# clayjohn/godot-volumetric-cloud-demo-v2

Measured on AMD Instinct MI355X. Metric: Mrays/s + hemisphere fps, 2048x1024 @ 128x6 steps, 1/2/4/8 MI355X, higher is better.
Workload: dtype f32

## Files before the change

godot-volumetric-cloud-demo-v2_amd/csrc/api.cpp:

```cpp
#include <cstdarg>
#include <cstdio>
#include <cstdlib>
#include <cstring>
#include <new>
#include <algorithm>
#include <vector>
#include "context.h"
#include "bake_core.h"
#include "mip_args.h"
#include "cloud_core.h"
#include "order_core.h"
#include "primitives_core.h"

using namespace csky;

__attribute__((constructor)) static void csky_runtime_defaults() {
    const char* no = getenv("CSKY_NO_ENV");
    if (no && no[0] && no[0] != '0') return;
    if (!getenv("GPU_MAX_HW_QUEUES")) setenv("GPU_MAX_HW_QUEUES", "16", 0);
}

static_assert(sizeof(csky_cloud_params) == sizeof(CloudParams), "ABI struct mismatch");

namespace {
// ... 33 lines not shown
    hs.d.reset(); hs.h.reset();
    if ((rc = hs.d.alloc(c, px))) return rc;
    return hs.h.alloc(c, px * 8);
}

}

extern "C" {

int csky_abi_version(void) { return CSKY_ABI_VERSION; }

int csky_device_count(void) {
    int n = 0;
    if (hipGetDeviceCount(&n) != hipSuccess) return 0;
    return n;
}

const char* csky_last_error(const csky_ctx* ctx) { return ctx ? ctx->err : g_err; }
const char* csky_last_warning(const csky_ctx* ctx) { return ctx ? ctx->warn : ""; }

int csky_create(csky_ctx** out, int device_id) {
    if (!out) return fail(nullptr, CSKY_ERR_INVALID, "csky_create: out is NULL");
    *out = nullptr;
    int n = 0;
    hipError_t e = hipGetDeviceCount(&n);
    if (e != hipSuccess || n <= 0)
        return fail(nullptr, CSKY_ERR_NO_DEVICE, "csky_create: no HIP device available (%s); libcloudsky has no CPU fallback",
                    e == hipSuccess ? "device count is 0" : hipGetErrorString(e));
    if (device_id < 0 || device_id >= n) return fail(nullptr, CSKY_ERR_INVALID, "csky_create: device_id %d out of range [0,%d)", device_id, n);
    csky_ctx* c = new (std::nothrow) csky_ctx();
    if (!c) return fail(nullptr, CSKY_ERR_INVALID, "csky_create: out of host memory");
    c->device = device_id;
    if (const int rc = create_resources(c)) { fail(nullptr, rc, "csky_create: %s", c->err); csky_destroy(c); return rc; }
    { int cus = 0; (void)hipDeviceGetAttribute(&cus, hipDeviceAttributeMultiprocessorCount, device_id); c->resident_wgs = (cus > 0 ? cus : 256) * cloud_resident_workgroups_per_cu(); }
    if (const char* pe = getenv("CSKY_PERSISTENT")) c->persistent = atoi(pe);
    if (const char* pe = getenv("CSKY_PERSISTENT_WGS")) { const int n = atoi(pe); if (n > 0) c->resident_wgs = n; }
    *out = c;
    return CSKY_OK;
}

void csky_destroy(csky_ctx* c) {
    if (!c) return;
    (void)hipSetDevice(c->device);
    (void)hipDeviceSynchronize();
    delete c;
}

#ifdef CSKY_BRICK_BOUND
static int upload_brick_bounds(csky_ctx* c, const uint8_t* large_rgba8) {
    std::vector<float> tab(16 * 16 * 16);
    for (int bz = 0; bz < 16; bz++) for (int by = 0; by < 16; by++) for (int bx = 0; bx < 16; bx++) {
        int rm = 0, fm = 1 << 30;
        for (int z = bz * 8; z <= bz * 8 + 8; z++) for (int y = by * 8; y <= by * 8 + 8; y++) for (int x = bx * 8; x <= bx * 8 + 8; x++) {
            const uint8_t* tx = large_rgba8 + ((((size_t)(z & 127) * 128 + (y & 127)) * 128 + (x & 127)) * 4);
            rm = std::max(rm, (int)tx[0]); fm = std::min(fm, 5 * tx[1] + 2 * tx[2] + tx[3]);
        }
        const float r = rm * (1.0f / 255.0f), f = fm * (1.0f / (8.0f * 255.0f));
        tab[((size_t)bz * 16 + by) * 16 + bx] = (r + (1.0f - f)) / (2.0f - f) * 1.000004f;
    }
    if (const int rc = c->noise.d_brick.grow(c, tab.size())) return rc;
    HIPCHK(c, hipMemcpy(c->noise.d_brick, tab.data(), tab.size() * sizeof(float), hipMemcpyHostToDevice));
    return CSKY_OK;
}
#endif

static int set_noise(csky_ctx* c, const uint8_t* large_rgba8, const uint8_t* small_rgb8, const uint8_t* weather_rgb8, bool chains_given) {
    if (!c) return fail(nullptr, CSKY_ERR_INVALID, "csky_set_noise: ctx is NULL");
    if (!large_rgba8 || !small_rgb8 || !weather_rgb8) return fail(c, CSKY_ERR_INVALID, "csky_set_noise: NULL texture pointer");
    int rc; if ((rc = bind(c))) return rc;
// ... 445 lines not shown
```

godot-volumetric-cloud-demo-v2_amd/csrc/cloud_kernels.hip:

```cpp
#include <hip/hip_runtime.h>
#include "kernels.h"
#include "cloud_core.h"
#include "order_core.h"
#include <type_traits>
#pragma clang fp contract(off)

namespace csky {

constexpr int QCAP = 96;
constexpr int QSTEPS = 48;
constexpr int Q_FLOATS = 5 * QCAP + 7 * QCAP + 3 * QSTEPS;

__device__ __forceinline__ void wave_lds_fence() {
    __builtin_amdgcn_fence(__ATOMIC_RELEASE, "wavefront");
    __builtin_amdgcn_wave_barrier();
    __builtin_amdgcn_fence(__ATOMIC_ACQUIRE, "wavefront");
}

__device__ __forceinline__ float ray_phase(const FrameConsts& fc, const Ray& ray) {
    float phase = 0.0f;
    if (ray.above) {
        const float ct = fc.ldir[0] * ray.dx + fc.ldir[1] * ray.dy + fc.ldir[2] * ray.dz;
        phase = fmaxf(fmaxf(henyey_greenstein(ct, 0.6f), henyey_greenstein(ct, fc.hg_g2)), henyey_greenstein(ct, -0.2f));
    }
// ... 71 lines not shown
        }
        if (count <= QCAP - 64 && cs < QSTEPS && i + 1 < step_end) continue;
        if (count == 0) continue;
        wave_lds_fence();
        light_march_batch(T, fc, ls, count, lane, [&](int k, float& x, float& y, float& z) { x = ev_px[k]; y = ev_py[k]; z = ev_pz[k]; }, ev_lt, QCAP);
        wave_lds_fence();
        for (int s = 0; s < cs; s++) {
            const unsigned lo = st_lo[s], hi = st_hi[s];
            const bool mine = lane < 32 ? ((lo >> lane) & 1u) : ((hi >> (lane - 32)) & 1u);
            if (mine) {
                const int slot = (int)st_base[s] + (int)__builtin_amdgcn_mbcnt_hi(hi, __builtin_amdgcn_mbcnt_lo(lo, 0u));
                float cd = 0.0f;
                for (int j = 0; j < nl; j++) cd += ev_lt[j * QCAP + slot];
                const float et = ev_t[slot], ehf = ev_hf[slot];
                const float dt = fast_exp(nd * et * ray.ss);
                shade_sample(fc, phase, et, ehf, dt, cd, Tr, alpha, Lr, Lg, Lb);
                o.incloud++;
            }
        }
        wave_lds_fence();
        count = 0; cs = 0;
        if (fc.early_eps > 0.0f) {
            if (Tr < fc.early_eps) live = false;
            if (!__any(live)) break;
        }
    }
    o.r = Lr; o.g = Lg; o.b = Lb; o.a = sat(alpha); o.t = Tr;
    return o;
}

constexpr int CQ_CAP = 128;
constexpr int CQ_STEPS = 66;
constexpr int CQ_FLOATS = 5 * CQ_CAP + CQ_CAP / 4 + 3 * CQ_STEPS + 2 + 128 + 320;

#ifndef CSKY_EAGER_LIGHT
#define CSKY_EAGER_LIGHT 1
#endif
#if CSKY_EAGER_LIGHT
#define CSKY_LIGHT_SAMPLE(CT) sample_density_eager<true, false, CT>
#else
#define CSKY_LIGHT_SAMPLE(CT) sample_density<CT>
#endif
#ifndef CSKY_EAGER_PRIMARY
#define CSKY_EAGER_PRIMARY 0
#endif
#if CSKY_EAGER_PRIMARY == 1
#define CSKY_PRIMARY_SAMPLE(CT) sample_density_eager<false, false, CT>
#elif CSKY_EAGER_PRIMARY == 2
#define CSKY_PRIMARY_SAMPLE(CT) sample_density_eager<true, false, CT>
#else
#define CSKY_PRIMARY_SAMPLE(CT) sample_density<CT>
#endif
#ifndef CSKY_LIGHT_STRAIGHT
#define CSKY_LIGHT_STRAIGHT 1
#endif
#if CSKY_EAGER_LIGHT
template <int CT, int J, class TS>
__device__ __forceinline__ void light_samples_from(const TS& T, const FrameConsts& fc, const int ls, float& lx, float& ly, float& lz, float& cd) {
    if constexpr (J < 6) {
        if (J >= ls) return;
        advance(lx, ly, lz, fc.linc[J][0], fc.linc[J][1], fc.linc[J][2]);
        const float lhf = height_fraction(length3_shell(lx, ly, lz));
        cd += sample_density_eager<true, (J > 2), CT>(T, fc, lx, ly, lz, lhf, fc.wpos_x, fc.wpos_y, J > 2 ? J - 2 : 0, J);
        light_samples_from<CT, J + 1>(T, fc, ls, lx, ly, lz, cd);
    }
}
// ... 14 lines not shown
        for (int j = 0; j < JS; j++) {
            if (j >= ls) break;
            advance(lx, ly, lz, fc.linc[j][0], fc.linc[j][1], fc.linc[j][2]);
            const float lhf = height_fraction(length3_shell(lx, ly, lz));
            cd += CSKY_LIGHT_SAMPLE(CT)(T, fc, lx, ly, lz, lhf, fc.wpos_x, fc.wpos_y, j > 2 ? j - 2 : 0, j);
        }
    }
#if CSKY_EAGER_LIGHT
    if constexpr (STRAIGHT) {
        light_samples_from<CT, 0>(T, fc, ls, lx, ly, lz, cd);
    } else if constexpr (TS::small_detail) {
#pragma unroll 1
        for (int j = JS; j < 6; j++) {
            if (j >= ls) break;
            advance(lx, ly, lz, fc.linc[j][0], fc.linc[j][1], fc.linc[j][2]);
            const float lhf = height_fraction(length3_shell(lx, ly, lz));
            cd += sample_density_eager<true, true, CT>(T, fc, lx, ly, lz, lhf, fc.wpos_x, fc.wpos_y, j - 2, j);
        }
    }
#endif
    {
        lx = ex; ly = ey; lz = ez;
        advance(lx, ly, lz, fc.ldist[0], fc.ldist[1], fc.ldist[2]);
        const float lhf = height_fraction(length3_shell(lx, ly, lz));
        const float ld = CSKY_LIGHT_SAMPLE(CT)(T, fc, lx, ly, lz, lhf, 0.0f, 0.0f, 3, 5);
        cd += fast_pow(ld, (1.0f - lhf) * 0.8f + 0.5f);
    }
    float et, ehf, ess, eph;
    late(et, ehf, ess, eph);
    dt = fast_exp(nd * et * ess);
    shade_terms(fc, eph, et, ehf, dt, cd, Dr, Dg, Db, rq);
}

template <bool WHOLE, bool TALLY, int CT = 0, class TS, bool RISING = true>
__device__ __forceinline__ MarchOut march_compact(const TS& T, const FrameConsts& fc, Ray ray, float* __restrict__ q, int step_begin, int step_end) {
    constexpr bool SAT = WHOLE && !TS::cell32;
    constexpr bool DEAD = SAT && !TALLY;
    float* __restrict__ ev_px = q;
    float* __restrict__ ev_py = q + CQ_CAP;
    float* __restrict__ ev_pz = q + 2 * CQ_CAP;
    float* __restrict__ ev_t = q + 3 * CQ_CAP;
    float* __restrict__ ev_hf = q + 4 * CQ_CAP;
    unsigned char* __restrict__ ev_owner = reinterpret_cast<unsigned char*>(q + 5 * CQ_CAP);
    unsigned* __restrict__ st_lo = reinterpret_cast<unsigned*>(q + 5 * CQ_CAP + CQ_CAP / 4);
    unsigned* __restrict__ st_hi = st_lo + CQ_STEPS;
    unsigned* __restrict__ st_base = st_hi + CQ_STEPS;

    MarchOut o; o.r = o.g = o.b = o.a = 0.0f; o.t = 1.0f; o.incloud = 0;
    const int lane = threadIdx.x & 63;
    const int ls = fc.light_steps;
    const float phase = ray_phase(fc, ray);
    float px = ray.px, py = ray.py, pz = ray.pz;
    const float nd = -fc.density;
    bool live = ray.above;
    int count = 0, cs = 0;
    bool latched = false;
    unsigned skipped = 0u;
    unsigned* __restrict__ tally = st_base + CQ_STEPS;
    if constexpr (TALLY) { if (lane == 0) tally[0] = 0u; }
    float* __restrict__ ray_ss = reinterpret_cast<float*>(tally + 2);
    float* __restrict__ ray_ph = ray_ss + 64;
    ray_ss[lane] = ray.ss; ray_ph[lane] = phase;
    float* __restrict__ acc = ray_ph + 64;
    acc[lane] = 1.0f; acc[64 + lane] = 0.0f; acc[128 + lane] = 0.0f; acc[192 + lane] = 0.0f; acc[256 + lane] = 0.0f;
    if (__builtin_amdgcn_ballot_w64(live) == 0ull) return o;
    for (int i = 0; i < step_begin; i++) advance(px, py, pz, ray.sx, ray.sy, ray.sz);
    int end = step_end;
    for (int i = step_begin;;) {
        if (i < end) {
            float t, hf;
            bool have = false, below_top = false;
            if (live) {
                advance(px, py, pz, ray.sx, ray.sy, ray.sz);
                hf = height_fraction(length3_shell(px, py, pz));
                t = CSKY_PRIMARY_SAMPLE(CT)(T, fc, px, py, pz, hf, fc.wpos_x, fc.wpos_y, 0, 0);
                have = t > 0.0f;
                below_top = !(hf >= fc.hf_hi);
            }
            if constexpr (SAT && TALLY) {
                skipped += (unsigned)__popcll(__builtin_amdgcn_ballot_w64(have && latched));
                have = have && !latched;
            }
            if constexpr (RISING) {
                if ((i & 3) == 3 && __builtin_amdgcn_ballot_w64(below_top) == 0ull) end = i + 1;
            } else {
                if ((i & 3) == 3 && __builtin_amdgcn_ballot_w64(live) == 0ull) end = i + 1;
            }
            const unsigned long long m = __builtin_amdgcn_ballot_w64(have);
            if (m != 0ull) {
                const int slot = count + (int)__builtin_amdgcn_mbcnt_hi((unsigned)(m >> 32), __builtin_amdgcn_mbcnt_lo((unsigned)m, 0u));
                if (have) { ev_px[slot] = px; ev_py[slot] = py; ev_pz[slot] = pz; ev_t[slot] = t; ev_hf[slot] = hf; ev_owner[slot] = (unsigned char)lane; }
                if (lane == 0) { st_lo[cs] = (unsigned)m; st_hi[cs] = (unsigned)(m >> 32); st_base[cs] = (unsigned)count; }
                count += __popcll(m);
                cs++;
            }
            i++;
        }
        const bool last = i >= end;
        if (count == 0) { if (last) break; continue; }
        if (count < 64 && !last) continue;
        wave_lds_fence();
        const int n = count < 64 ? count : 64;
        unsigned long long carry = 0ull;
        if constexpr (TALLY) { if (lane == 0) tally[0] += (unsigned)n; }
        if (lane < n) {
            float Dr, Dg, Db, rq, dt;
            light_march_terms<CT>(T, fc, ls, nd, ev_px[lane], ev_py[lane], ev_pz[lane],
                              [&](float& et, float& ehf, float& ess, float& eph) { et = ev_t[lane]; ehf = ev_hf[lane]; const int ow = ev_owner[lane]; ess = ray_ss[ow]; eph = ray_ph[ow]; }, Dr, Dg, Db, rq, dt);
            ev_px[lane] = Dr; ev_py[lane] = Dg; ev_pz[lane] = Db; ev_t[lane] = rq; ev_hf[lane] = dt;
        }
        wave_lds_fence();
        float Tr = acc[lane], alpha = acc[64 + lane], Lr = acc[128 + lane], Lg = acc[192 + lane], Lb = acc[256 + lane];
        for (int s = 0; s < cs; s++) {
            const unsigned lo = (unsigned)__builtin_amdgcn_readfirstlane((int)st_lo[s]), hi = (unsigned)__builtin_amdgcn_readfirstlane((int)st_hi[s]);
            const bool mine = __builtin_amdgcn_inverse_ballot_w64(((unsigned long long)hi << 32) | lo);
            const int slot = (int)st_base[s] + (int)__builtin_amdgcn_mbcnt_hi(hi, __builtin_amdgcn_mbcnt_lo(lo, 0u));
            if (mine && slot < n) {
                composite_sample(ev_hf[slot], ev_t[slot], ev_px[slot], ev_py[slot], ev_pz[slot], Tr, alpha, Lr, Lg, Lb);
            }
            if (s == cs - 1) carry = __builtin_amdgcn_ballot_w64(mine && slot >= n);
        }
        if constexpr (DEAD) {
            const bool cand = live && alpha >= SAT_ALPHA_MIN;
            if (fc.sat_skip != 0 && __builtin_amdgcn_ballot_w64(cand) != 0ull) {
                float B[3];
                ray_saturation_bound(fc, ray_ph[lane], B);
                const float L[3] = {Lr, Lg, Lb};
                if (cand && ray_saturated(fc, Tr, alpha, L, B)) live = false;
            }
        } else if constexpr (SAT) {
            const bool cand = !latched && alpha >= SAT_ALPHA_MIN;
            if (fc.sat_skip != 0 && __builtin_amdgcn_ballot_w64(cand) != 0ull) {
                float B[3];
                ray_saturation_bound(fc, ray_ph[lane], B);
                const float L[3] = {Lr, Lg, Lb};
                latched = latched || (cand && ray_saturated(fc, Tr, alpha, L, B));
            }
        }
        acc[lane] = Tr; acc[64 + lane] = alpha; acc[128 + lane] = Lr; acc[192 + lane] = Lg; acc[256 + lane] = Lb;
        wave_lds_fence();
        const int rem = count - n;
        if (rem > 0) {
            float a0 = 0.0f, a1 = 0.0f, a2 = 0.0f, a3 = 0.0f, a4 = 0.0f; unsigned char a5 = 0;
            if (lane < rem) { a0 = ev_px[n + lane]; a1 = ev_py[n + lane]; a2 = ev_pz[n + lane]; a3 = ev_t[n + lane]; a4 = ev_hf[n + lane]; a5 = ev_owner[n + lane]; }
            wave_lds_fence();
            if (lane < rem) { ev_px[lane] = a0; ev_py[lane] = a1; ev_pz[lane] = a2; ev_t[lane] = a3; ev_hf[lane] = a4; ev_owner[lane] = a5; }
            if (lane == 0) { st_lo[0] = (unsigned)carry; st_hi[0] = (unsigned)(carry >> 32); st_base[0] = 0u; }
            wave_lds_fence();
            count = rem; cs = 1;
        } else {
            count = 0; cs = 0;
        }
        if (fc.early_eps > 0.0f) {
            if (Tr < fc.early_eps) live = false;
            if (__builtin_amdgcn_ballot_w64(live) == 0ull) break;
        }
        if (last && count == 0) break;
    }
    wave_lds_fence();
    o.r = acc[128 + lane]; o.g = acc[192 + lane]; o.b = acc[256 + lane]; o.a = sat(acc[64 + lane]); o.t = acc[lane];
    if constexpr (TALLY) o.incloud = lane == 0 ? tally[0] + skipped : 0u;
    return o;
}


struct Pixel { int gx, gy, lr; bool valid; };
__device__ __forceinline__ Pixel footprint_pixel(const RenderGeom& G, const uint32_t logical, const int tiles_x, const int bw, const int tile, const int lane) {
    const int local_rows = G.n_bands * G.band_rows;
    const int slab = (int)logical / tiles_x, bx = (int)logical - slab * tiles_x;
    Pixel p;
    p.gx = bx * bw + tile * 8 + (lane & 7);
    p.lr = slab * 8 + (lane >> 3);
    p.valid = p.gx < G.tile_w && p.lr < local_rows;
    const int band = p.lr / G.band_rows, rib = p.lr - band * G.band_rows;
    p.gy = (G.first_band + band * G.band_stride) * G.band_rows + rib;
    return p;
}
__device__ __forceinline__ void store_pixel(uint2* __restrict__ out, const RenderGeom& G, int gx, int gy, int lr, float r, float g, float b, float a) {
    out[(size_t)(G.out_full ? gy : lr) * G.pitch_px + gx] = pack_half4(f2h(r), f2h(g), f2h(b), f2h(a));
}
// ... 122 lines not shown
    {
        const uint4* __restrict__ src = reinterpret_cast<const uint4*>(T.detail_h);
        uint4* dst = reinterpret_cast<uint4*>(lds_all);
        for (int i = threadIdx.x; i < DETAIL_FLOATS / 4; i += 1024) dst[i] = src[i];
    }
    __syncthreads();
    const uint32_t logical = order[blockIdx.x];
    if (logical == 0xffffffffu) return;
    const int wave = threadIdx.x >> 6, lane = threadIdx.x & 63;
    const Pixel pix = footprint_pixel(G, logical, (G.tile_w + 127) >> 7, 128, wave, lane);
    const bool valid = pix.valid;
    const FrameConsts& fc = *fcp;
    Ray ray = ray_setup(fc, valid ? pix.gx : 0, valid ? pix.gy : 0);
    if (!valid) ray.above = false;
    TexSet Tl = T;
    Tl.detail_lds = detail_s;
    const MarchOut o = march_queue(Tl, fc, ray, queues + wave * Q_FLOATS, 0, fc.primary_steps);
    if (valid) {
        store_pixel(out, G, pix.gx, pix.gy, pix.lr, o.r, o.g, o.b, o.a);
    }
    if (stats || wg_cost) {
        unsigned ic = o.incloud, ab = ray.above ? 1u : 0u;
        for (int off = 32; off > 0; off >>= 1) { ic += __shfl_down(ic, off); ab += __shfl_down(ab, off); }
        if (lane == 0) {
            if (stats) { atomicAdd(&stats[0], (unsigned long long)ic); atomicAdd(&stats[1], (unsigned long long)ab); }
            if (wg_cost) atomicAdd(&wg_cost[logical], ic + 16u * ab);
        }
    }
}

#ifndef CSKY_COMPACT_WAVES
#define CSKY_COMPACT_WAVES 7
#endif
template <int VARIANT, int SEG, class TS = TexSet, bool TALLY = true, int CT = 0>
__device__ __forceinline__ void render_block(TS T, const FrameConsts* __restrict__ fcp, const RenderGeom& G, const uint32_t logical, const uint32_t rec,
                                             uint2* __restrict__ out, unsigned long long* __restrict__ stats, uint32_t* __restrict__ wg_cost, const int tile_of_wave = -1) {
    constexpr int BW = 32 / SEG;
    const int tiles_x = (G.tile_w + BW - 1) / BW;
    const int local_rows = G.n_bands * G.band_rows;
    const int slab = (int)logical / tiles_x, bx = (int)logical - slab * tiles_x;
    const int wave = threadIdx.x >> 6, lane = threadIdx.x & 63;
    const int tile = tile_of_wave >= 0 ? tile_of_wave : wave / SEG, seg = tile_of_wave >= 0 ? 0 : wave - tile * SEG;
    const int gx = bx * BW + tile * 8 + (lane & 7);
    const int lr = slab * 8 + (lane >> 3);
    const bool valid = gx < G.tile_w && lr < local_rows;
    const int band = lr / G.band_rows, rib = lr - band * G.band_rows;
    const int gy = (G.first_band + band * G.band_stride) * G.band_rows + rib;

    const FrameConsts& fc = *fcp;
    T.detail_lds = nullptr;
    Ray ray = ray_setup(fc, valid ? gx : 0, valid ? gy : 0);
    if (!valid) ray.above = false;
    MarchOut o;
    if constexpr (VARIANT == 0) {
        static_assert(SEG == 1, "the lock-step reference variant marches whole rays");
        o = march(T, fc, ray);
    } else {
        __shared__ float lds[4][VARIANT == 3 ? CQ_FLOATS : Q_FLOATS];
        const int s0 = (fc.primary_steps * seg) / SEG, s1 = (fc.primary_steps * (seg + 1)) / SEG;
        if constexpr (VARIANT == 3) o = march_compact<SEG == 1, TALLY, CT>(T, fc, ray, &lds[wave][0], s0, s1);
        else o = march_queue(T, fc, ray, &lds[wave][0], s0, s1);
        if constexpr (SEG > 1) {
            __shared__ float comb[4][5][64];
            comb[wave][0][lane] = o.r; comb[wave][1][lane] = o.g; comb[wave][2][lane] = o.b; comb[wave][3][lane] = o.t; comb[wave][4][lane] = o.a;
            __syncthreads();
            if (seg == 0) {
                float Tr = o.t, na = 1.0f - o.a;
#pragma unroll
                for (int s = 1; s < SEG; s++) {
                    const int w = tile * SEG + s;
                    o.r += Tr * comb[w][0][lane]; o.g += Tr * comb[w][1][lane]; o.b += Tr * comb[w][2][lane];
                    Tr *= comb[w][3][lane]; na *= 1.0f - comb[w][4][lane];
                }
                o.a = sat(1.0f - na); o.t = Tr;
            }
        }
    }
    if (valid && seg == 0) {
        store_pixel(out, G, gx, gy, lr, o.r, o.g, o.b, o.a);
    }
    if constexpr (TALLY) {
    if (stats || wg_cost) {
        unsigned ic = o.incloud, ab = (ray.above && seg == 0) ? 1u : 0u;
        for (int off = 32; off > 0; off >>= 1) { ic += __shfl_down(ic, off); ab += __shfl_down(ab, off); }
        if (lane == 0) {
            if (stats) { atomicAdd(&stats[0], (unsigned long long)ic); atomicAdd(&stats[1], (unsigned long long)ab); }
            if (wg_cost) atomicAdd(&wg_cost[logical], ic + 16u * ab);
        }
    }
    }
}

template <int VARIANT, int SEG, class TS = TexSet, bool TALLY = true>
__global__ __launch_bounds__(256, VARIANT == 3 ? CSKY_COMPACT_WAVES : 7) void clouds_kernel(TS T, const FrameConsts* __restrict__ fcp, RenderGeom G, const uint32_t* __restrict__ order,
                                                     uint2* __restrict__ out, unsigned long long* __restrict__ stats, uint32_t* __restrict__ wg_cost) {
    const uint32_t logical = order[blockIdx.x];
    if (logical == 0xffffffffu) return;
    render_block<VARIANT, SEG, TS, TALLY>(T, fcp, G, logical, blockIdx.x, out, stats, wg_cost);
}

template <int VARIANT, bool TALLY = true, int CT = 0>
__global__ __launch_bounds__(256, VARIANT == 3 ? CSKY_COMPACT_WAVES : 7) void clouds_kernel_persistent(TexSet T, const FrameConsts* __restrict__ fcp, RenderGeom G,
        const uint32_t* __restrict__ order, const uint32_t n_items, uint32_t* __restrict__ heads, uint2* __restrict__ out, unsigned long long* __restrict__ stats,
        uint32_t* __restrict__ wg_cost) {
    unsigned xcc;
    asm volatile("s_getreg_b32 %0, hwreg(HW_REG_XCC_ID)" : "=s"(xcc));
    xcc &= 7u;
    __shared__ uint32_t ticket, slot_ready[2], slot_reads[2], slot_entry[2], slot_rec[2];
    if (threadIdx.x == 0) { ticket = 0; slot_ready[0] = slot_ready[1] = 0; slot_reads[0] = slot_reads[1] = 0; }
    static_assert(VARIANT == 3, "the persistent form exists for the compact march only: its light march is the one that reads the table");
    __shared__ __attribute__((aligned(16))) uint4 det_small[TexSetSmallDetail::SMALL_DETAIL_CELLS];
    if (threadIdx.x < (unsigned)TexSetSmallDetail::SMALL_DETAIL_CELLS) det_small[threadIdx.x] = T.detail[detail_level_offset(TexSetSmallDetail::SMALL_DETAIL_FIRST) + threadIdx.x];
    __syncthreads();
    const bool lane0 = (threadIdx.x & 63) == 0;
    for (;;) {
        uint32_t tv = 0;
        if (lane0) tv = __hip_atomic_fetch_add(&ticket, 1u, __ATOMIC_RELAXED, __HIP_MEMORY_SCOPE_WORKGROUP);
        const uint32_t t = (uint32_t)__builtin_amdgcn_readfirstlane((int)tv);
        const uint32_t f = t >> 2, sl = f & 1u;
        const int tile = (int)(t & 3u);
        uint32_t logical = 0xfffffffeu, rec = 0;
        if (tile == 0) {
            for (unsigned k = 0; k < 8u; k++) {
                const unsigned y = (xcc + k) & 7u;
                uint32_t jv = 0;
                if (lane0) jv = atomicAdd(&heads[y], 1u);
                const uint32_t j = (uint32_t)__builtin_amdgcn_readfirstlane((int)jv);
                uint32_t i;
                if (persistent_pop_index(j, y, n_items, i)) { logical = order[i]; rec = i; break; }
            }
            for (;;) {
                const uint32_t r = (uint32_t)__builtin_amdgcn_readfirstlane((int)__hip_atomic_load(&slot_reads[sl], __ATOMIC_ACQUIRE, __HIP_MEMORY_SCOPE_WORKGROUP));
                if (r == 3u * (f >> 1)) break;
                __builtin_amdgcn_s_sleep(1);
            }
            if (lane0) {
                slot_entry[sl] = logical; slot_rec[sl] = rec;
                __hip_atomic_store(&slot_ready[sl], f + 1u, __ATOMIC_RELEASE, __HIP_MEMORY_SCOPE_WORKGROUP);
            }
        } else {
            for (;;) {
                const uint32_t r = (uint32_t)__builtin_amdgcn_readfirstlane((int)__hip_atomic_load(&slot_ready[sl], __ATOMIC_ACQUIRE, __HIP_MEMORY_SCOPE_WORKGROUP));
                if (r == f + 1u) break;
                __builtin_amdgcn_s_sleep(1);
            }
            logical = (uint32_t)__builtin_amdgcn_readfirstlane((int)slot_entry[sl]);
            rec = (uint32_t)__builtin_amdgcn_readfirstlane((int)slot_rec[sl]);
            if (lane0) __hip_atomic_fetch_add(&slot_reads[sl], 1u, __ATOMIC_RELEASE, __HIP_MEMORY_SCOPE_WORKGROUP);
        }
        if (logical == 0xfffffffeu) {
            if (lane0 && atomicAdd(&heads[8], 1u) == gridDim.x * 4u - 1u) {
                for (unsigned k = 0; k < 9u; k++) atomicExch(&heads[k], 0u);
            }
            return;
        }
        if (logical != 0xffffffffu) {
            TexSetSmallDetail Ts;
            static_cast<TexSet&>(Ts) = T;
            Ts.det_small = (SmallDetailTable)det_small;
            render_block<VARIANT, 1, TexSetSmallDetail, TALLY, CT>(Ts, fcp, G, logical, rec, out, stats, wg_cost, tile);
        }
    }
}


__global__ __launch_bounds__(256) void lpt_hist_kernel(const uint32_t* __restrict__ cost, int n, int shift, uint32_t* __restrict__ hist) {
    const int i = blockIdx.x * 256 + threadIdx.x;
    if (i < n) atomicAdd(&hist[lpt_bucket(cost[i], shift)], 1u);
}
__global__ __launch_bounds__(LPT_BUCKETS) void lpt_scan_kernel(uint32_t* __restrict__ hist, uint32_t* __restrict__ offsets) {
    __shared__ uint32_t sh[LPT_BUCKETS];
    const int t = threadIdx.x;
    const uint32_t own = hist[t];
    hist[t] = 0u;
    sh[t] = own;
    __syncthreads();
    for (int off = 1; off < LPT_BUCKETS; off <<= 1) {
        const uint32_t v = t >= off ? sh[t - off] : 0u;
        __syncthreads();
        sh[t] += v;
        __syncthreads();
    }
    offsets[t] = sh[t] - own;
}
__global__ __launch_bounds__(256) void lpt_scatter_kernel(uint32_t* __restrict__ cost, int n, int shift, uint32_t* __restrict__ offsets,
                                                          uint32_t* __restrict__ order) {
    const int i = blockIdx.x * 256 + threadIdx.x;
    if (i < n) {
        order[atomicAdd(&offsets[lpt_bucket(cost[i], shift)], 1u)] = (uint32_t)i;
        cost[i] = 0u;
    }
}
hipError_t launch_lpt_order(uint32_t* d_cost, int n, int shift, uint32_t* d_scratch, uint32_t* d_order, hipStream_t s) {
// ... 14 lines not shown
    static_order_kernel<<<(grid + 255) / 256, 256, 0, s>>>(mode, tiles_x, slabs, grid, d_order);
    return hipGetLastError();
}

__global__ __launch_bounds__(256) void interleave_bands_kernel(const uint4* __restrict__ src, size_t member_stride16, int members, uint32_t band16, uint32_t total_bands,
                                                              uint4* __restrict__ dst) {
    const size_t total = (size_t)band16 * total_bands;
    for (size_t i = (size_t)blockIdx.x * 256 + threadIdx.x; i < total; i += (size_t)gridDim.x * 256) {
        const uint32_t k = (uint32_t)(i / band16), c = (uint32_t)(i - (size_t)k * band16);
        dst[i] = src[(size_t)(k % members) * member_stride16 + (size_t)(k / members) * band16 + c];
    }
}
hipError_t launch_interleave_bands(const void* d_gathered, size_t member_stride_bytes, int members, size_t band_bytes, int total_bands, void* d_frame, hipStream_t s) {
    const size_t chunks = band_bytes / 16 * (size_t)total_bands;
    if (!chunks) return hipSuccess;
    const unsigned grid = (unsigned)(chunks / 256 + 1 < 48 ? chunks / 256 + 1 : 48);
    interleave_bands_kernel<<<grid, 256, 0, s>>>(reinterpret_cast<const uint4*>(d_gathered), member_stride_bytes / 16, members, (uint32_t)(band_bytes / 16), (uint32_t)total_bands,
                                                 reinterpret_cast<uint4*>(d_frame));
    return hipGetLastError();
}

__global__ __launch_bounds__(256) void sqrt_shell_kernel(const float* __restrict__ in, float* __restrict__ out, size_t n) {
    const size_t i = (size_t)blockIdx.x * 256 + threadIdx.x;
    if (i < n) out[i] = sqrt_shell(in[i]);
}
hipError_t launch_sqrt_shell(const float* d_in, float* d_out, size_t n, hipStream_t s) {
    if (n == 0) return hipSuccess;
    sqrt_shell_kernel<<<(unsigned)((n + 255) / 256), 256, 0, s>>>(d_in, d_out, n);
    return hipGetLastError();
}

static const char* const kVariantNames[] = {"lockstep", "queue", "queue-lds", "compact"};
int cloud_resident_workgroups_per_cu() { return CSKY_COMPACT_WAVES; }
int cloud_variant_count() { return (int)(sizeof(kVariantNames) / sizeof(kVariantNames[0])); }
const char* cloud_variant_name(int v) { return (v >= 0 && v < cloud_variant_count()) ? kVariantNames[v] : nullptr; }

hipError_t launch_clouds(int variant, int seg, const TexSet& t, const FrameConsts* d_fc, const RenderGeom& g, const uint32_t* d_order, int grid,
                         uint2* d_out, unsigned long long* d_stats, uint32_t* d_wg_cost, hipStream_t s, uint32_t* d_heads, int resident, const TexSet32* t32, bool census_lean,
                         int ct_mode) {
    if (grid <= 0) return hipSuccess;
    if (ct_mode < 0 || ct_mode > 2) return hipErrorInvalidValue;
    const bool tally = (d_stats != nullptr || d_wg_cost != nullptr) && !census_lean;
    if (t32) {
        if (variant != 3 || seg != 1) return hipErrorInvalidValue;
        clouds_kernel<3, 1, TexSet32><<<grid, 256, 0, s>>>(*t32, d_fc, g, d_order, d_out, d_stats, d_wg_cost);
        return hipGetLastError();
    }
    if (d_heads && variant == 3 && seg == 1) {
        const unsigned n = (unsigned)(grid < resident ? grid : resident);
        const auto go = [&](auto tl, auto ct) {
            clouds_kernel_persistent<3, decltype(tl)::value, decltype(ct)::value><<<n, 256, 0, s>>>(t, d_fc, g, d_order, (uint32_t)grid, d_heads, d_out, d_stats, d_wg_cost);
        };
        const auto with_mode = [&](auto tl) {
            if (ct_mode == 1) go(tl, std::integral_constant<int, 1>());
            else if (ct_mode == 2) go(tl, std::integral_constant<int, 2>());
            else go(tl, std::integral_constant<int, 0>());
        };
        if (tally) with_mode(std::true_type()); else with_mode(std::false_type());
        return hipGetLastError();
    }
    if (variant == 0 && seg == 1) clouds_kernel<0, 1><<<grid, 256, 0, s>>>(t, d_fc, g, d_order, d_out, d_stats, d_wg_cost);
    else if (variant == 1 && seg == 1) clouds_kernel<1, 1><<<grid, 256, 0, s>>>(t, d_fc, g, d_order, d_out, d_stats, d_wg_cost);
    else if (variant == 1 && seg == 2) clouds_kernel<1, 2><<<grid, 256, 0, s>>>(t, d_fc, g, d_order, d_out, d_stats, d_wg_cost);
    else if (variant == 1 && seg == 4) clouds_kernel<1, 4><<<grid, 256, 0, s>>>(t, d_fc, g, d_order, d_out, d_stats, d_wg_cost);
    else if (variant == 3 && seg == 1 && tally) clouds_kernel<3, 1, TexSet, true><<<grid, 256, 0, s>>>(t, d_fc, g, d_order, d_out, d_stats, d_wg_cost);
    else if (variant == 3 && seg == 1) clouds_kernel<3, 1, TexSet, false><<<grid, 256, 0, s>>>(t, d_fc, g, d_order, d_out, d_stats, d_wg_cost);
    else if (variant == 3 && seg == 2) clouds_kernel<3, 2><<<grid, 256, 0, s>>>(t, d_fc, g, d_order, d_out, d_stats, d_wg_cost);
    else if (variant == 3 && seg == 4) clouds_kernel<3, 4><<<grid, 256, 0, s>>>(t, d_fc, g, d_order, d_out, d_stats, d_wg_cost);
    else if ((variant == 1 || variant == 3) && seg == 5) {
        hipError_t e = hipFuncSetAttribute(reinterpret_cast<const void*>(&clouds_kernel_interleaved<0>), hipFuncAttributeMaxDynamicSharedMemorySize,
                                           (int)(IL_BLOCK_FLOATS * sizeof(float)));
        if (e != hipSuccess) return e;
        clouds_kernel_interleaved<0><<<grid, 256, IL_BLOCK_FLOATS * sizeof(float), s>>>(t, d_fc, g, d_order, d_out, d_stats, d_wg_cost);
    }
    else if (variant == 2) {
        constexpr size_t bytes = ((DETAIL_CHAIN_TEXELS + 7) / 8 * 4 + 16 * Q_FLOATS) * sizeof(float);
        hipError_t e = hipFuncSetAttribute(reinterpret_cast<const void*>(&clouds_kernel_lds<0>), hipFuncAttributeMaxDynamicSharedMemorySize, (int)bytes);
        if (e != hipSuccess) return e;
        clouds_kernel_lds<0><<<grid, 1024, bytes, s>>>(t, d_fc, g, d_order, d_out, d_stats, d_wg_cost);
    }
    else return hipErrorInvalidValue;
    return hipGetLastError();
}
// ... 217 lines not shown
```

godot-volumetric-cloud-demo-v2_amd/csrc/clouds_launch.cpp:

```cpp
#include <cstring>
#include "context.h"
#include "launch_policy.h"
#include "order_core.h"

namespace csky {

TexSet texset(const csky_ctx* c) {
    const NoiseSet& n = c->noise;
    TexSet t;
#ifdef CSKY_BRICK_BOUND
    t.brick = n.d_brick;
#endif
    t.shape = n.d_shape; t.detail = n.d_detail; t.weather = n.d_weather; t.sky = c->lut.cur_f(); t.sky_w = c->lut.aw; t.sky_h = c->lut.ah; t.detail_lod5 = n.st.detail_lod5(); t.detail_h = n.d_detail_h; t.detail_lds = nullptr;
    return t;
}

TexSet32 texset32(const csky_ctx* c) {
    TexSet32 t;
    static_cast<TexSet&>(t) = texset(c);
    t.shape32 = c->noise.d_shape32; t.detail32 = c->noise.d_detail32; t.weather32 = c->noise.d_weather32;
    return t;
}

namespace {
// ... 39 lines not shown
    if (!c->noise.st.have()) return fail(c, CSKY_ERR_STATE, "render_clouds: csky_set_noise has not been called");
    if (c->lut.st.holds == SkyLutHolds::None) return fail(c, CSKY_ERR_STATE, "render_clouds: no sky LUT yet (call csky_render_sky_lut first; cloud_sky.gd:187,242)");
    if (!(p->texture_size[0] >= 1.0f) || !(p->texture_size[1] >= 1.0f)) return fail(c, CSKY_ERR_INVALID, "render_clouds: texture_size must be >= 1");
    int rc; if ((rc = check_bands(c, b, tile_w))) return rc;
    if (pitch_bytes % 8 || pitch_bytes < (size_t)tile_w * 8) return fail(c, CSKY_ERR_INVALID, "render_clouds: row pitch must be a multiple of 8 and >= tile_w*8");
    if (b->n_bands == 0) return CSKY_OK;
    CloudParams cp; memcpy(&cp, p, sizeof cp);
    if (setup && (rc = frame_setup(c, cp, s))) return rc;
    RenderGeom g; g.tile_w = tile_w; g.band_rows = b->band_rows; g.first_band = b->first_band; g.band_stride = b->band_stride; g.n_bands = b->n_bands;
    g.pitch_px = (uint32_t)(pitch_bytes / 8); g.out_full = out_full ? 1 : 0;
    const long long waves = ((long long)(tile_w + 7) / 8) * (((long long)b->n_bands * b->band_rows + 7) / 8);
    const LaunchPlan pl = plan_launch({c->variant, c->noise.st.cell32(), c->segments, c->sched_mode, c->frames_overlapping, c->persistent}, waves);
    const int tiles_x = (g.tile_w + pl.bw - 1) / pl.bw, slabs = (g.n_bands * g.band_rows + 7) >> 3, nblocks = tiles_x * slabs;
    FrameRing& ring = c->ring;
    const int slot = ring.cur;
    uint32_t* const heads = pl.persist ? ring.heads(slot) : nullptr;
    TexSet32 t32; const TexSet32* t32p = nullptr;
    if (c->noise.st.cell32()) { t32 = texset32(c); t32p = &t32; }
    const Event* kt = nullptr;
    if (c->kt.on && (rc = c->kt.next_pair(c, kt))) return rc;
    if ((rc = ensure_order(c, slot, pl.static_mode, tiles_x, slabs, s))) return rc;
    const uint32_t* order = ring.slot[slot].order;
    int grid = ring.slot[slot].order_st.grid();
    uint32_t* cost = nullptr;
    if (pl.feedback) {
        if ((rc = ring.reserve_feedback(c, (size_t)(grid > nblocks ? grid : nblocks)))) return rc;
        cost = ring.cost(slot);
        const FeedbackKey fkey = feedback_key(g.tile_w, g.band_rows, g.first_band, g.band_stride, g.n_bands, cp.texture_size, cp.update_position, pl.mode, pl.static_mode, pl.seg);
        if (ring.slot[slot].feedback.begin(fkey)) { order = ring.feedback_order(slot); grid = nblocks; }
    }
    if (kt) HIPCHK(c, hipEventRecord(kt[0], s));
    {
        const hipError_t le = launch_clouds(pl.variant, pl.seg, texset(c), ring.fc(), g, order, grid, d_out, d_stats, cost, s, heads, c->resident_wgs, t32p, c->census_lean,
                                                setup_args(c, cp).ct_mode);
        if (le != hipSuccess) { if (heads) (void)hipMemsetAsync(heads, 0, 16 * sizeof(uint32_t), s); return fail(c, CSKY_ERR_HIP, "cloud kernel launch failed: %s", hipGetErrorString(le)); }
    }
    if (kt) HIPCHK(c, hipEventRecord(kt[1], s));
    if (pl.feedback) {
        HIPCHK(c, launch_lpt_order(cost, nblocks, lpt_shift(c->primary_steps), ring.sort_scratch(slot), ring.feedback_order(slot), s));
        ring.slot[slot].feedback.sort_enqueued();
    }
    return ring.march_enqueued(c, slot, s);
}

}
```

godot-volumetric-cloud-demo-v2_amd/csrc/context.h:

```cpp
#pragma once
#include <hip/hip_runtime_api.h>
#include <cmath>
#include <cstddef>
#include <cstdint>
#include <vector>
#include "../../include/cloudsky_internal.h"
#include "kernels.h"
#include "owners.h"
#include "frame_ring.h"
#include "host_stage.h"
#include "noise_set.h"
#include "sky_lut_reuse.h"

constexpr int RING = 8;
constexpr int HOST_RING = 8;

namespace csky {

struct SkyLut {
    SkyLutHeld st;
    DevBuf<uint16_t> ring_h[2]; DevBuf<float4> ring_f[2];
    int cur = 0;
    int aw = 0, ah = 0;
    std::vector<hipEvent_t> writers;
// ... 104 lines not shown
            float ms = 0.0f;
            HIPCHK(c, hipEventElapsedTime(&ms, ev[(size_t)i * 2], ev[(size_t)i * 2 + 1]));
            sum += ms;
        }
        *total_ms = sum; *launches = count; count = 0;
        return CSKY_OK;
    }
};

}

struct csky_ctx {
    int device = 0;
    csky::Stream stream;
    csky::HostStage stage;
    csky::Event ev0, ev1, ev_copy;
    csky::NoiseSet noise;
    bool use_window = true;
    csky::DevBuf<uint16_t> d_trans_h; csky::DevBuf<float4> d_trans_f; int tw = 0, th = 0; bool have_trans = false;
    int tlut = CSKY_TLUT_REFERENCE;
    csky::SkyLut lut;
    csky::RowsCache rows_cache;
    csky::FrameRing ring;
    csky::DevBuf<unsigned long long> d_stats;
    csky::DevBuf<uint2> d_frame;
    int primary_steps = 128, light_steps = 6;
    float early_eps = 0.0f;
    int variant = CSKY_DEFAULT_VARIANT;
    int sched_mode = -1;
    int segments = 0;
    int frames_in_flight = 1;
    int frames_overlapping = 1;
    int persistent = 1; int resident_wgs = 0;
    csky::TimingPool kt;
    struct RadSet { csky::DevBuf<float4> tab, src_cones, out_cones;
                    int cones_ss = 0, cones_s = 0; int S = 0, L = 0, Ss = 0; bool valid = false; };
    RadSet rad, rad_pf;
    csky::Event ev_rad;
    csky_cloud_stats last_stats = {0, 0, 0};
    bool shadow_exact_end = true;
    csky::Event ev_aerial;
    csky::DevBuf<csky::FrameConsts> d_rays_fc;
    csky::Event ev_rays; bool rays_pending = false;
    bool census_lean = false;
    struct HostSlot { csky::Stream s; csky::Event done; csky::DevBuf<uint2> d; csky::PinnedBuf h; long long ticket = -1; int w = 0, hh = 0; bool busy = false; };
    HostSlot hring[HOST_RING]; int hslots = 2; long long next_ticket = 0;
    char err[512] = {0};
    char warn[512] = {0};
};

namespace csky {

extern thread_local char g_err[512];

inline int bind(csky_ctx* c) { HIPCHK(c, hipSetDevice(c->device)); return CSKY_OK; }
inline hipStream_t stream_of(const csky_ctx* c, void* hip_stream) { return hip_stream ? (hipStream_t)hip_stream : (hipStream_t)c->stream; }
inline HostCall host_call(csky_ctx* c, const char* fn, std::initializer_list<size_t> bytes) { return HostCall(c, c->stage, c->stream, fn, bytes); }
inline int launched(csky_ctx* c, const char* fn, hipError_t e) { return e == hipSuccess ? CSKY_OK : fail(c, CSKY_ERR_HIP, "%s: kernel launch failed: %s", fn, hipGetErrorString(e)); }
inline int view_check(csky_ctx* c, const char* fn, const csky_view* view) {
    for (int k = 0; k < 9; k++) if (!std::isfinite(view->basis[k])) return fail(c, CSKY_ERR_INVALID, "%s: the view's basis is not finite", fn);
    if (!(view->fov_y_degrees > 0.0f && view->fov_y_degrees < 180.0f)) return fail(c, CSKY_ERR_INVALID, "%s: fov_y_degrees must be in (0, 180)", fn);
    return CSKY_OK;
}

int host_slot_prepare(csky_ctx* c, csky_ctx::HostSlot& hs, size_t px);

// ... 15 lines not shown
```

godot-volumetric-cloud-demo-v2_amd/csrc/kernels.h:

```cpp
#pragma once
#include <hip/hip_runtime_api.h>
#include "csky_common.h"
#include "composite_core.h"
#include "noise_core.h"

namespace csky {

hipError_t launch_transmittance(int w, int h, uint16_t* d_half, float4* d_float, hipStream_t s, int tlut = 0);
hipError_t launch_sky_lut(int w, int h, const float sun[3], const float4* d_trans, int tw, int th, uint16_t* d_half,
                          float4* d_float, hipStream_t s, int tlut = 0);
hipError_t launch_sky_lut_rows(int w, int h, int row0, int row_stride, const float sun[3], const float4* d_trans, int tw, int th, uint2* d_rows, float4* d_whole_f,
                               hipStream_t s, int tlut = 0);
hipError_t launch_composite(const CompositeArgs& a, uint2* d_out, hipStream_t s, int tlut = 0);
struct SetupArgs {
    int primary_steps, light_steps;
    float early_eps, hf_lo, hf_hi;
    int ct_mode, sat_skip;
};
hipError_t launch_frame_setup(const CloudParams& p, const float4* d_sky, int sw, int sh, const SetupArgs& a, FrameConsts* d_fc, hipStream_t s);
hipError_t launch_frame_setup_taps(const CloudParams& p, const float sun[3], const float4* d_trans, int tw, int th, int sw, int sh, const SetupArgs& a, FrameConsts* d_fc,
                                   hipStream_t s, int tlut = 0);

hipError_t launch_shape_noise(uint32_t seed, int n, const ShapeNoiseParams& P, uint32_t* d_out, hipStream_t s);
hipError_t launch_detail_noise(uint32_t seed, int n, uint8_t* d_out, hipStream_t s);
hipError_t launch_mip_chain(uint8_t* d_chain, int n, int ch, int levels, hipStream_t s);
hipError_t launch_bake(const uint8_t* d_large_chain, const uint8_t* d_small_chain, const uint8_t* d_weather, ShapeTexel* d_shape, uint4* d_detail, uint16_t* d_detail_h,
                       uint4* d_weather_out, unsigned long long* d_inexact, int* d_range, hipStream_t s);
hipError_t launch_bake32(const uint8_t* d_large_chain, const uint8_t* d_small_chain, const uint8_t* d_weather, float4* d_shape32, float4* d_detail32, float4* d_weather32, hipStream_t s);

hipError_t launch_clouds(int variant, int seg, const TexSet& t, const FrameConsts* d_fc, const RenderGeom& g, const uint32_t* d_order, int grid,
                         uint2* d_out, unsigned long long* d_stats, uint32_t* d_wg_cost, hipStream_t s, uint32_t* d_heads = nullptr, int resident = 0,
                         const TexSet32* t32 = nullptr, bool census_lean = false,
                         int ct_mode = 0);
int cloud_resident_workgroups_per_cu();
int cloud_variant_count();
const char* cloud_variant_name(int v);
hipError_t launch_lpt_order(uint32_t* d_cost, int n, int shift, uint32_t* d_scratch, uint32_t* d_order, hipStream_t s);
hipError_t launch_static_order(int mode, int tiles_x, int slabs, int grid, uint32_t* d_order, hipStream_t s);
hipError_t launch_interleave_bands(const void* d_gathered, size_t member_stride_bytes, int members, size_t band_bytes, int total_bands, void* d_frame, hipStream_t s);
hipError_t launch_sqrt_shell(const float* d_in, float* d_out, size_t n, hipStream_t s);
struct RaysGeom;
hipError_t launch_clouds_rays(const TexSet& t, const TexSet32* t32, const FrameConsts* d_fc, const RaysGeom& g, const float* d_dirs, uint2* d_out, hipStream_t s);
struct ViewUpdateGeom;
hipError_t launch_clouds_view_update(const TexSet& t, const TexSet32* t32, const FrameConsts* d_fc, const ViewUpdateGeom& g, const uint2* d_prev, uint2* d_out, hipStream_t s);
struct ObserverGeom;
hipError_t launch_clouds_observer(const TexSet& t, const TexSet32* t32, const FrameConsts* d_fc, const ObserverGeom& g, const float* d_dirs, uint2* d_out, hipStream_t s);
struct SceneDepthGeom;
hipError_t launch_clouds_observer_depth(const TexSet& t, const TexSet32* t32, const FrameConsts* d_fc, const SceneDepthGeom& g, const float* d_dirs, const float* d_depth,
                                        uint2* d_out, hipStream_t s);

struct ShadowConsts;
hipError_t launch_cloud_shadow(const TexSet& t, const TexSet32* t32, const FrameConsts& fc, const ShadowConsts& sc, uint16_t* d_out, hipStream_t s);

struct AerialGeom;
hipError_t launch_aerial(const AerialGeom& g, const float4* d_trans, int tw, int th, uint2* d_out, hipStream_t s, int tlut = 0);

struct ShaftsMap;
hipError_t launch_shafts(const AerialGeom& g, const ShaftsMap& m, const float4* d_trans, int tw, int th, uint2* d_out, hipStream_t s, int tlut = 0);

struct DepthConsts;
hipError_t launch_cloud_depth(const TexSet& t, const TexSet32* t32, const FrameConsts& fc, const DepthConsts& dc, uint2* d_out, hipStream_t s);
hipError_t launch_cloud_depth_rays(const TexSet& t, const TexSet32* t32, const FrameConsts& fc, const DepthConsts& dc, const RaysGeom& g, const float* d_dirs,
                                   uint2* d_out, hipStream_t s);

struct CloudAerialGeom;
hipError_t launch_cloud_aerial(const CloudAerialGeom& g, const float4* d_trans, int tw, int th, const uint2* d_cloud, const uint2* d_depth, uint2* d_out,
                               hipStream_t s, int tlut = 0);
// ... 15 lines not shown
```

Baseline: 1638.

## Slim compact-march LDS queue so persistent kernel fits eight workgroups per CU

```diff
diff --git a/godot-volumetric-cloud-demo-v2_amd/csrc/api.cpp b/godot-volumetric-cloud-demo-v2_amd/csrc/api.cpp
--- a/godot-volumetric-cloud-demo-v2_amd/csrc/api.cpp
+++ b/godot-volumetric-cloud-demo-v2_amd/csrc/api.cpp
@@ -89,9 +89,10 @@
     if (!c) return fail(nullptr, CSKY_ERR_INVALID, "csky_create: out of host memory");
     c->device = device_id;
     if (const int rc = create_resources(c)) { fail(nullptr, rc, "csky_create: %s", c->err); csky_destroy(c); return rc; }
-    { int cus = 0; (void)hipDeviceGetAttribute(&cus, hipDeviceAttributeMultiprocessorCount, device_id); c->resident_wgs = (cus > 0 ? cus : 256) * cloud_resident_workgroups_per_cu(); }
+    { int cus = 0; (void)hipDeviceGetAttribute(&cus, hipDeviceAttributeMultiprocessorCount, device_id); cus = cus > 0 ? cus : 256;
+      c->resident_wgs = cus * cloud_resident_workgroups_per_cu(); c->resident_wgs_slim = cus * cloud_resident_workgroups_per_cu_slim(); }
     if (const char* pe = getenv("CSKY_PERSISTENT")) c->persistent = atoi(pe);
-    if (const char* pe = getenv("CSKY_PERSISTENT_WGS")) { const int n = atoi(pe); if (n > 0) c->resident_wgs = n; }
+    if (const char* pe = getenv("CSKY_PERSISTENT_WGS")) { const int n = atoi(pe); if (n > 0) c->resident_wgs = c->resident_wgs_slim = n; }
     *out = c;
     return CSKY_OK;
 }
diff --git a/godot-volumetric-cloud-demo-v2_amd/csrc/cloud_kernels.hip b/godot-volumetric-cloud-demo-v2_amd/csrc/cloud_kernels.hip
--- a/godot-volumetric-cloud-demo-v2_amd/csrc/cloud_kernels.hip
+++ b/godot-volumetric-cloud-demo-v2_amd/csrc/cloud_kernels.hip
@@ -127,6 +127,17 @@
 constexpr int CQ_CAP = 128;
 constexpr int CQ_STEPS = 66;
 constexpr int CQ_FLOATS = 5 * CQ_CAP + CQ_CAP / 4 + 3 * CQ_STEPS + 2 + 128 + 320;
+constexpr int CQ_HF_SLIM = 64;
+template <bool SLIM> struct ReplayBase {
+    __device__ __forceinline__ int first(const unsigned* __restrict__ st_base, int s) const { return (int)st_base[s]; }
+    __device__ __forceinline__ void next(unsigned, unsigned) {}
+};
+template <> struct ReplayBase<true> {
+    int base = 0;
+    __device__ __forceinline__ int first(const unsigned* __restrict__, int) const { return base; }
+    __device__ __forceinline__ void next(unsigned lo, unsigned hi) { base += __builtin_popcount(lo) + __builtin_popcount(hi); }
+};
+constexpr int CQ_FLOATS_SLIM = 4 * CQ_CAP + CQ_HF_SLIM + CQ_CAP / 4 + 2 * CQ_STEPS + 2 + 128 + 320;
 
 #ifndef CSKY_EAGER_LIGHT
 #define CSKY_EAGER_LIGHT 1
@@ -207,7 +218,7 @@
     shade_terms(fc, eph, et, ehf, dt, cd, Dr, Dg, Db, rq);
 }
 
-template <bool WHOLE, bool TALLY, int CT = 0, class TS, bool RISING = true>
+template <bool WHOLE, bool TALLY, int CT = 0, class TS, bool RISING = true, bool SLIM = false>
 __device__ __forceinline__ MarchOut march_compact(const TS& T, const FrameConsts& fc, Ray ray, float* __restrict__ q, int step_begin, int step_end) {
     constexpr bool SAT = WHOLE && !TS::cell32;
     constexpr bool DEAD = SAT && !TALLY;
@@ -216,8 +227,9 @@
     float* __restrict__ ev_pz = q + 2 * CQ_CAP;
     float* __restrict__ ev_t = q + 3 * CQ_CAP;
     float* __restrict__ ev_hf = q + 4 * CQ_CAP;
-    unsigned char* __restrict__ ev_owner = reinterpret_cast<unsigned char*>(q + 5 * CQ_CAP);
-    unsigned* __restrict__ st_lo = reinterpret_cast<unsigned*>(q + 5 * CQ_CAP + CQ_CAP / 4);
+    constexpr int HF_CAP = SLIM ? CQ_HF_SLIM : CQ_CAP;
+    unsigned char* __restrict__ ev_owner = reinterpret_cast<unsigned char*>(q + (4 * CQ_CAP + HF_CAP));
+    unsigned* __restrict__ st_lo = reinterpret_cast<unsigned*>(q + (4 * CQ_CAP + HF_CAP) + CQ_CAP / 4);
     unsigned* __restrict__ st_hi = st_lo + CQ_STEPS;
     unsigned* __restrict__ st_base = st_hi + CQ_STEPS;
 
@@ -231,7 +243,7 @@
     int count = 0, cs = 0;
     bool latched = false;
     unsigned skipped = 0u;
-    unsigned* __restrict__ tally = st_base + CQ_STEPS;
+    unsigned* __restrict__ tally = st_base + (SLIM ? 0 : CQ_STEPS);
     if constexpr (TALLY) { if (lane == 0) tally[0] = 0u; }
     float* __restrict__ ray_ss = reinterpret_cast<float*>(tally + 2);
     float* __restrict__ ray_ph = ray_ss + 64;
@@ -264,8 +276,13 @@
             const unsigned long long m = __builtin_amdgcn_ballot_w64(have);
             if (m != 0ull) {
                 const int slot = count + (int)__builtin_amdgcn_mbcnt_hi((unsigned)(m >> 32), __builtin_amdgcn_mbcnt_lo((unsigned)m, 0u));
+                if constexpr (SLIM) {
+                    if (have) { ev_px[slot] = px; ev_py[slot] = py; ev_pz[slot] = pz; ev_t[slot] = t; ev_owner[slot] = (unsigned char)lane; if (slot < CQ_HF_SLIM) ev_hf[slot] = hf; }
+                    if (lane == 0) { st_lo[cs] = (unsigned)m; st_hi[cs] = (unsigned)(m >> 32); }
+                } else {
                 if (have) { ev_px[slot] = px; ev_py[slot] = py; ev_pz[slot] = pz; ev_t[slot] = t; ev_hf[slot] = hf; ev_owner[slot] = (unsigned char)lane; }
                 if (lane == 0) { st_lo[cs] = (unsigned)m; st_hi[cs] = (unsigned)(m >> 32); st_base[cs] = (unsigned)count; }
+                }
                 count += __popcll(m);
                 cs++;
             }
@@ -286,10 +303,12 @@
         }
         wave_lds_fence();
         float Tr = acc[lane], alpha = acc[64 + lane], Lr = acc[128 + lane], Lg = acc[192 + lane], Lb = acc[256 + lane];
+        ReplayBase<SLIM> sb;
         for (int s = 0; s < cs; s++) {
             const unsigned lo = (unsigned)__builtin_amdgcn_readfirstlane((int)st_lo[s]), hi = (unsigned)__builtin_amdgcn_readfirstlane((int)st_hi[s]);
             const bool mine = __builtin_amdgcn_inverse_ballot_w64(((unsigned long long)hi << 32) | lo);
-            const int slot = (int)st_base[s] + (int)__builtin_amdgcn_mbcnt_hi(hi, __builtin_amdgcn_mbcnt_lo(lo, 0u));
+            const int slot = sb.first(st_base, s) + (int)__builtin_amdgcn_mbcnt_hi(hi, __builtin_amdgcn_mbcnt_lo(lo, 0u));
+            sb.next(lo, hi);
             if (mine && slot < n) {
                 composite_sample(ev_hf[slot], ev_t[slot], ev_px[slot], ev_py[slot], ev_pz[slot], Tr, alpha, Lr, Lg, Lb);
             }
@@ -317,10 +336,15 @@
         const int rem = count - n;
         if (rem > 0) {
             float a0 = 0.0f, a1 = 0.0f, a2 = 0.0f, a3 = 0.0f, a4 = 0.0f; unsigned char a5 = 0;
+            if constexpr (SLIM) {
+                if (lane < rem) { a0 = ev_px[n + lane]; a1 = ev_py[n + lane]; a2 = ev_pz[n + lane]; a3 = ev_t[n + lane]; a5 = ev_owner[n + lane]; a4 = height_fraction(length3_shell(a0, a1, a2)); }
+            } else {
             if (lane < rem) { a0 = ev_px[n + lane]; a1 = ev_py[n + lane]; a2 = ev_pz[n + lane]; a3 = ev_t[n + lane]; a4 = ev_hf[n + lane]; a5 = ev_owner[n + lane]; }
+            }
             wave_lds_fence();
             if (lane < rem) { ev_px[lane] = a0; ev_py[lane] = a1; ev_pz[lane] = a2; ev_t[lane] = a3; ev_hf[lane] = a4; ev_owner[lane] = a5; }
-            if (lane == 0) { st_lo[0] = (unsigned)carry; st_hi[0] = (unsigned)(carry >> 32); st_base[0] = 0u; }
+            if constexpr (SLIM) { if (lane == 0) { st_lo[0] = (unsigned)carry; st_hi[0] = (unsigned)(carry >> 32); } }
+            else { if (lane == 0) { st_lo[0] = (unsigned)carry; st_hi[0] = (unsigned)(carry >> 32); st_base[0] = 0u; } }
             wave_lds_fence();
             count = rem; cs = 1;
         } else {
@@ -509,7 +533,11 @@
 #ifndef CSKY_COMPACT_WAVES
 #define CSKY_COMPACT_WAVES 7
 #endif
-template <int VARIANT, int SEG, class TS = TexSet, bool TALLY = true, int CT = 0>
+#ifndef CSKY_PERSISTENT_SLIM_WAVES
+#define CSKY_PERSISTENT_SLIM_WAVES 8
+#endif
+constexpr bool persistent_slim(int variant, bool tally, int ct) { return variant == 3 && !tally && ct != 0; }
+template <int VARIANT, int SEG, class TS = TexSet, bool TALLY = true, int CT = 0, bool SLIM = false>
 __device__ __forceinline__ void render_block(TS T, const FrameConsts* __restrict__ fcp, const RenderGeom& G, const uint32_t logical, const uint32_t rec,
                                              uint2* __restrict__ out, unsigned long long* __restrict__ stats, uint32_t* __restrict__ wg_cost, const int tile_of_wave = -1) {
     constexpr int BW = 32 / SEG;
@@ -533,9 +561,10 @@
         static_assert(SEG == 1, "the lock-step reference variant marches whole rays");
         o = march(T, fc, ray);
     } else {
-        __shared__ float lds[4][VARIANT == 3 ? CQ_FLOATS : Q_FLOATS];
+        static_assert(!SLIM || (VARIANT == 3 && SEG == 1), "the slim queue is the compact whole-ray march's");
+        __shared__ float lds[4][VARIANT == 3 ? (SLIM ? CQ_FLOATS_SLIM : CQ_FLOATS) : Q_FLOATS];
         const int s0 = (fc.primary_steps * seg) / SEG, s1 = (fc.primary_steps * (seg + 1)) / SEG;
-        if constexpr (VARIANT == 3) o = march_compact<SEG == 1, TALLY, CT>(T, fc, ray, &lds[wave][0], s0, s1);
+        if constexpr (VARIANT == 3) o = march_compact<SEG == 1, TALLY, CT, TS, true, SLIM>(T, fc, ray, &lds[wave][0], s0, s1);
         else o = march_queue(T, fc, ray, &lds[wave][0], s0, s1);
         if constexpr (SEG > 1) {
             __shared__ float comb[4][5][64];
@@ -577,7 +606,7 @@
 }
 
 template <int VARIANT, bool TALLY = true, int CT = 0>
-__global__ __launch_bounds__(256, VARIANT == 3 ? CSKY_COMPACT_WAVES : 7) void clouds_kernel_persistent(TexSet T, const FrameConsts* __restrict__ fcp, RenderGeom G,
+__global__ __launch_bounds__(256, persistent_slim(VARIANT, TALLY, CT) ? CSKY_PERSISTENT_SLIM_WAVES : VARIANT == 3 ? CSKY_COMPACT_WAVES : 7) void clouds_kernel_persistent(TexSet T, const FrameConsts* __restrict__ fcp, RenderGeom G,
         const uint32_t* __restrict__ order, const uint32_t n_items, uint32_t* __restrict__ heads, uint2* __restrict__ out, unsigned long long* __restrict__ stats,
         uint32_t* __restrict__ wg_cost) {
     unsigned xcc;
@@ -587,6 +616,9 @@
     if (threadIdx.x == 0) { ticket = 0; slot_ready[0] = slot_ready[1] = 0; slot_reads[0] = slot_reads[1] = 0; }
     static_assert(VARIANT == 3, "the persistent form exists for the compact march only: its light march is the one that reads the table");
     __shared__ __attribute__((aligned(16))) uint4 det_small[TexSetSmallDetail::SMALL_DETAIL_CELLS];
+    constexpr bool SLIM = persistent_slim(VARIANT, TALLY, CT);
+    static_assert(!SLIM || 4 * CQ_FLOATS_SLIM * sizeof(float) + 9 * sizeof(uint32_t) + sizeof(det_small) <= 163840 / CSKY_PERSISTENT_SLIM_WAVES,
+                  "the specialised persistent forms no longer fit eight workgroups into a CU's LDS");
     if (threadIdx.x < (unsigned)TexSetSmallDetail::SMALL_DETAIL_CELLS) det_small[threadIdx.x] = T.detail[detail_level_offset(TexSetSmallDetail::SMALL_DETAIL_FIRST) + threadIdx.x];
     __syncthreads();
     const bool lane0 = (threadIdx.x & 63) == 0;
@@ -635,7 +667,7 @@
             TexSetSmallDetail Ts;
             static_cast<TexSet&>(Ts) = T;
             Ts.det_small = (SmallDetailTable)det_small;
-            render_block<VARIANT, 1, TexSetSmallDetail, TALLY, CT>(Ts, fcp, G, logical, rec, out, stats, wg_cost, tile);
+            render_block<VARIANT, 1, TexSetSmallDetail, TALLY, CT, SLIM>(Ts, fcp, G, logical, rec, out, stats, wg_cost, tile);
         }
     }
 }
@@ -716,12 +748,22 @@
 
 static const char* const kVariantNames[] = {"lockstep", "queue", "queue-lds", "compact"};
 int cloud_resident_workgroups_per_cu() { return CSKY_COMPACT_WAVES; }
+int cloud_resident_workgroups_per_cu_slim() {
+    int per_cu = CSKY_PERSISTENT_SLIM_WAVES;
+    const void* const forms[2] = {reinterpret_cast<const void*>(&clouds_kernel_persistent<3, false, 1>), reinterpret_cast<const void*>(&clouds_kernel_persistent<3, false, 2>)};
+    for (const void* f : forms) {
+        int n = 0;
+        if (hipOccupancyMaxActiveBlocksPerMultiprocessor(&n, f, 256, 0) != hipSuccess || n <= 0) { (void)hipGetLastError(); n = CSKY_COMPACT_WAVES; }
+        if (n < per_cu) per_cu = n;
+    }
+    return per_cu;
+}
 int cloud_variant_count() { return (int)(sizeof(kVariantNames) / sizeof(kVariantNames[0])); }
 const char* cloud_variant_name(int v) { return (v >= 0 && v < cloud_variant_count()) ? kVariantNames[v] : nullptr; }
 
 hipError_t launch_clouds(int variant, int seg, const TexSet& t, const FrameConsts* d_fc, const RenderGeom& g, const uint32_t* d_order, int grid,
                          uint2* d_out, unsigned long long* d_stats, uint32_t* d_wg_cost, hipStream_t s, uint32_t* d_heads, int resident, const TexSet32* t32, bool census_lean,
-                         int ct_mode) {
+                         int ct_mode, int resident_slim) {
     if (grid <= 0) return hipSuccess;
     if (ct_mode < 0 || ct_mode > 2) return hipErrorInvalidValue;
     const bool tally = (d_stats != nullptr || d_wg_cost != nullptr) && !census_lean;
@@ -731,8 +773,9 @@
         return hipGetLastError();
     }
     if (d_heads && variant == 3 && seg == 1) {
-        const unsigned n = (unsigned)(grid < resident ? grid : resident);
         const auto go = [&](auto tl, auto ct) {
+            const int res = persistent_slim(3, decltype(tl)::value, decltype(ct)::value) && resident_slim > 0 ? resident_slim : resident;
+            const unsigned n = (unsigned)(grid < res ? grid : res);
             clouds_kernel_persistent<3, decltype(tl)::value, decltype(ct)::value><<<n, 256, 0, s>>>(t, d_fc, g, d_order, (uint32_t)grid, d_heads, d_out, d_stats, d_wg_cost);
         };
         const auto with_mode = [&](auto tl) {
diff --git a/godot-volumetric-cloud-demo-v2_amd/csrc/clouds_launch.cpp b/godot-volumetric-cloud-demo-v2_amd/csrc/clouds_launch.cpp
--- a/godot-volumetric-cloud-demo-v2_amd/csrc/clouds_launch.cpp
+++ b/godot-volumetric-cloud-demo-v2_amd/csrc/clouds_launch.cpp
@@ -95,7 +95,7 @@
     if (kt) HIPCHK(c, hipEventRecord(kt[0], s));
     {
         const hipError_t le = launch_clouds(pl.variant, pl.seg, texset(c), ring.fc(), g, order, grid, d_out, d_stats, cost, s, heads, c->resident_wgs, t32p, c->census_lean,
-                                                setup_args(c, cp).ct_mode);
+                                                setup_args(c, cp).ct_mode, c->resident_wgs_slim);
         if (le != hipSuccess) { if (heads) (void)hipMemsetAsync(heads, 0, 16 * sizeof(uint32_t), s); return fail(c, CSKY_ERR_HIP, "cloud kernel launch failed: %s", hipGetErrorString(le)); }
     }
     if (kt) HIPCHK(c, hipEventRecord(kt[1], s));
diff --git a/godot-volumetric-cloud-demo-v2_amd/csrc/context.h b/godot-volumetric-cloud-demo-v2_amd/csrc/context.h
--- a/godot-volumetric-cloud-demo-v2_amd/csrc/context.h
+++ b/godot-volumetric-cloud-demo-v2_amd/csrc/context.h
@@ -160,6 +160,7 @@
     int frames_in_flight = 1;
     int frames_overlapping = 1;
     int persistent = 1; int resident_wgs = 0;
+    int resident_wgs_slim = 0;
     csky::TimingPool kt;
     struct RadSet { csky::DevBuf<float4> tab, src_cones, out_cones;
                     int cones_ss = 0, cones_s = 0; int S = 0, L = 0, Ss = 0; bool valid = false; };
diff --git a/godot-volumetric-cloud-demo-v2_amd/csrc/kernels.h b/godot-volumetric-cloud-demo-v2_amd/csrc/kernels.h
--- a/godot-volumetric-cloud-demo-v2_amd/csrc/kernels.h
+++ b/godot-volumetric-cloud-demo-v2_amd/csrc/kernels.h
@@ -31,8 +31,10 @@
 hipError_t launch_clouds(int variant, int seg, const TexSet& t, const FrameConsts* d_fc, const RenderGeom& g, const uint32_t* d_order, int grid,
                          uint2* d_out, unsigned long long* d_stats, uint32_t* d_wg_cost, hipStream_t s, uint32_t* d_heads = nullptr, int resident = 0,
                          const TexSet32* t32 = nullptr, bool census_lean = false,
-                         int ct_mode = 0);
+                         int ct_mode = 0,
+                         int resident_slim = 0);
 int cloud_resident_workgroups_per_cu();
+int cloud_resident_workgroups_per_cu_slim();
 int cloud_variant_count();
 const char* cloud_variant_name(int v);
 hipError_t launch_lpt_order(uint32_t* d_cost, int n, int shift, uint32_t* d_scratch, uint32_t* d_order, hipStream_t s);
```

New measurement: 1672, median of 6. 1.02x the previous value.
